# duyhominhnguyen/conan-fgw

Measured on AMD Instinct MI355X. Metric: molecules/s (K=5 conformers), higher is better.
Workload: dtype f32

## Files before the change

conan-fgw_amd/_lib.py:

```python
from __future__ import annotations

import ctypes
import os
import subprocess

import torch

_HERE = os.path.dirname(os.path.abspath(__file__))
_SO = os.path.join(_HERE, "libconan_fgw_hip.so")
_LIB = None
ABI_VERSION = 6

c_int, c_float, c_void_p, c_ll = ctypes.c_int, ctypes.c_float, ctypes.c_void_p, ctypes.c_longlong
f32, i32, i64 = torch.float32, torch.int32, torch.int64


def _c(t: torch.Tensor) -> torch.Tensor:
    return t if t.is_contiguous() else t.contiguous()


class FgwParams(ctypes.Structure):
    _fields_ = [("alpha", c_float), ("epsilon", c_float), ("max_iter", c_int), ("tol", c_float), ("inner_tol", c_float),
                ("num_iter_max", c_int), ("stop_thr", c_float), ("fixed_structure", c_int), ("fixed_features", c_int),
                ("warmstart", c_int), ("loss_fun", c_int), ("cs_small_int", c_int)]
# ... 149 lines not shown
    "conan_sinkhorn_bwd_lds_resident": (c_int, [c_int, c_int]),
    "conan_sinkhorn_bwd": (c_int, [_P] * 7 + [c_int, c_int, c_int, c_ll, c_float, c_int, c_int] + [_P] * 9),
    "conan_sinkhorn_ext_workspace_bytes": (c_ll, [c_int, c_int, c_int]),
    "conan_sinkhorn_ext_lds_resident": (c_int, [c_int, c_int]),
    "conan_sinkhorn_ext_nerr": (c_int, [c_int, c_int, c_int]),
    "conan_sinkhorn_ext_fwd": (c_int, [_P] * 7 + [c_int, c_int, c_int, c_ll, ctypes.c_double, c_int, c_int, ctypes.c_double, ctypes.c_double, c_int,
                                       ctypes.c_double, c_int] + [_P] * 11),
    "conan_fgw_barycenter_bwd": (c_int, [_P, _P, _P, _P, c_int, c_int, c_int, c_int, _P, _P]),
    "conan_fgw_barycenter_bwd_full_workspace_bytes": (c_ll, [c_int, c_int, c_int, c_int]),
    "conan_fgw_barycenter_bwd_full": (c_int, [_P, _P, _P, _P, _P, _P, _P, _P, _P, c_int, c_int, c_int, c_int, c_int, c_int, c_int,
                                              _P, _P, _P, _P, _P, _P, _P, _P]),
    "conan_fgw_readout_fwd": (c_int, [_P, c_int, c_int, c_int, c_int, c_int, _P, _P]),
    "conan_fgw_readout_bwd": (c_int, [_P, _P, c_int, c_int, c_int, c_int, c_int, _P, _P]),
}

_D = ctypes.c_double
EXT_SIGNATURES = {
    "conan_fgw_acc_pair_bwd_lds_resident": (c_int, [c_int]),
    "conan_fgw_acc_pair_bwd_workspace_bytes": (c_ll, [c_int, c_int, c_int]),
    "conan_fgw_acc_pair_bwd": (c_int, [_P] * 6 + [c_int, c_int, _D, _D, c_int] + [_P] * 12),
}

EXT_TABLES = {
    "conan_fgw_hip_pair_grad.h": {
        "conan_fgw_pair_bwd_lds_resident": (c_int, [c_int]),
        "conan_fgw_pair_bwd_workspace_bytes": (c_ll, [c_int, c_int, c_int, c_int]),
        "conan_fgw_pair_bwd": (c_int, [_P] * 6 + [c_int, c_int, _D, _D, c_int, c_int, _D, c_int, c_int] + [_P] * 13),
    },
    "conan_fgw_hip_bregman_grad.h": {
        "conan_fgw_bregman_bwd_lds_resident": (c_int, [c_int]),
        "conan_fgw_bregman_bwd_workspace_bytes": (c_ll, [c_int, c_int, c_int]),
        "conan_fgw_bregman_bwd": (c_int, [_P] * 6 + [c_int, c_int, _D, _D, c_int, c_int, c_int] + [_P] * 13),
    },
    "conan_fgw_hip_sinkhorn_hists.h": {
        "conan_sinkhorn_hists_max_hists": (c_int, [c_int, c_int]),
        "conan_sinkhorn_hists_lds_resident": (c_int, [c_int, c_int, c_int]),
        "conan_sinkhorn_hists_workspace_bytes": (c_ll, [c_int, c_int, c_int, c_int]),
        "conan_sinkhorn_hists_fwd": (c_int, [_P] * 8 + [c_int] * 4 + [c_ll, _D, c_int, _D] + [_P] * 7),
        "conan_sinkhorn_hists_loss_bwd": (c_int, [_P] * 7 + [c_int] * 4 + [c_ll, _D] + [_P] * 2),
    },
    "conan_fgw_hip_mixup_grad.h": {
        "conan_fgw_mixup_barycenter_fwd_record": (c_int, [_P] * 7 + [c_int, c_int, c_int, c_int, ctypes.POINTER(FgwParams), _D, c_int, _D] + [_P] * 9),
        "conan_fgw_mixup_barycenter_bwd_lds_resident": (c_int, [c_int]),
        "conan_fgw_mixup_barycenter_bwd_workspace_bytes": (c_ll, [c_int] * 5),
        "conan_fgw_mixup_barycenter_bwd": (c_int, [_P] * 6 + [c_int, c_int, c_int, c_int, ctypes.POINTER(FgwParams), _D, c_int, _D] + [_P] * 15),
    },
}

_ERR = {-1: "bad argument", -2: "HIP launch failure", -3: "unsupported configuration"}


def library_path() -> str:
    return _SO


def build(force: bool = False) -> str:
    args = ["make", "-C", os.path.join(_HERE, "csrc"), "-s", "-j8"]
    if force:
        args.append("-B")
    subprocess.check_call(args)
    return _SO


def lib():
    global _LIB
    if _LIB is None:
# ... 58 lines not shown
```

conan-fgw_amd/csrc/gemm.hip:

```cpp
#include "fp_planes.h"

namespace {

constexpr int BM = 64;
constexpr int BK = 32;
constexpr int XP = BK + 1;

template <int NB>
__global__ void __launch_bounds__(256) k_linear(const float *__restrict__ x, const float *__restrict__ w,
                                                const float *__restrict__ bias, const float *__restrict__ residual,
                                                int M, int K, int N, int w_kn, int act, float *__restrict__ y,
                                                const int *__restrict__ m_dev) {
    constexpr int BN = 64 * NB;
    if (m_dev) M = min(M, *m_dev);
    if ((int)blockIdx.x * BM >= M) return;
    constexpr int WP = BN + 1;
    __shared__ float xs[BM * XP];
    __shared__ float ws[BK * WP];
    const int tid = threadIdx.x, lane = tid & 63, wave = tid >> 6;
    const int wm = wave >> 1, wn = wave & 1;
    const int row0 = blockIdx.x * BM, col0 = blockIdx.y * BN;
    f32x16 acc[NB];
#pragma unroll
    for (int b = 0; b < NB; ++b)
#pragma unroll
        for (int r = 0; r < 16; ++r) acc[b][r] = 0.f;

    for (int k0 = 0; k0 < K; k0 += BK) {
        for (int t = tid; t < BM * BK; t += 256) {
            int r = t / BK, k = t % BK;
            int gr = row0 + r, gk = k0 + k;
            xs[r * XP + k] = (gr < M && gk < K) ? x[(size_t)gr * K + gk] : 0.f;
        }
// ... 167 lines not shown
                    if (act == 1) v = ssp_f(v);
                    if (act == 3) v = v / (1.0f + __expf(-v));
                    if (act == 2) v *= 1.0f - 0.5f * __expf(-rv[a][b][r]);
                    else if (residual) v += rv[a][b][r];
                    y[(size_t)gr * N + gc] = v;
                }
        }
    }
}

__global__ void k_ssp_bwd(const float *__restrict__ dy, const float *__restrict__ y, long long n, int width,
                          const int *__restrict__ m_dev, float *__restrict__ g) {
    if (m_dev) n = min(n, (long long)(*m_dev) * width);
    long long i = (long long)blockIdx.x * blockDim.x + threadIdx.x;
    const long long stride = (long long)gridDim.x * blockDim.x;
    for (; i < n; i += stride) g[i] = dy[i] * (1.0f - 0.5f * expf(-y[i]));
}

constexpr int WG_SLICES_MAX = 768;


__device__ __forceinline__ f32x16 wg_mma6(const bf16x8 &a1, const bf16x8 &a2, const bf16x8 &a3, const bf16x8 &b1, const bf16x8 &b2,
                                         const bf16x8 &b3, f32x16 acc) {
    acc = __builtin_amdgcn_mfma_f32_32x32x16_bf16(a3, b1, acc, 0, 0, 0);
    acc = __builtin_amdgcn_mfma_f32_32x32x16_bf16(a2, b2, acc, 0, 0, 0);
    acc = __builtin_amdgcn_mfma_f32_32x32x16_bf16(a1, b3, acc, 0, 0, 0);
    acc = __builtin_amdgcn_mfma_f32_32x32x16_bf16(a2, b1, acc, 0, 0, 0);
    acc = __builtin_amdgcn_mfma_f32_32x32x16_bf16(a1, b2, acc, 0, 0, 0);
    acc = __builtin_amdgcn_mfma_f32_32x32x16_bf16(a1, b1, acc, 0, 0, 0);
    return acc;
}


template <int KT, bool RBF, bool H16 = false>
__device__ __forceinline__ void wgrad_lds_body(const float *__restrict__ g, const float *__restrict__ x, int M, int K, int N,
                                               float *__restrict__ slabs, float *__restrict__ bias_slabs,
                                               const int *__restrict__ m_dev, const float *__restrict__ dist,
                                               const float *__restrict__ offset, float coeff, int slice, int num_slices, int tile_n, int tile_k,
                                               const float *__restrict__ gmax = nullptr) {
    constexpr int ROWS = 16, RG = ROWS / 8, W = 128 + KT, FRAGS = RG * W, NF = (FRAGS + 255) / 256;
    constexpr int TNB = KT == 128 ? 2 : 1;
    constexpr int NPL = H16 ? 2 : 3;
    static_assert(W % 64 == 0, "a wave's 64 fragments share one row group and one operand");
    __shared__ uint4 frag[2][NPL][RG][W];
    if (m_dev) M = min(M, *m_dev);
    float gsc = 1.0f, gun = 1.0f;
    if constexpr (H16) grad_scale(*gmax, 0.f, gsc, gun);
    const int tid = threadIdx.x, lane = tid & 63, wave = __builtin_amdgcn_readfirstlane(tid >> 6);
    const int l31 = lane & 31, h = lane >> 5;
    const int n0 = KT == 128 ? (wave >> 1) * 64 : wave * 32, k0 = KT == 128 ? (wave & 1) * 64 : 0;
    const int nb = tile_n * 128, kb = tile_k * KT;
    const int r_begin = slice * ROWS, r_end = M, STEP = num_slices * ROWS;
    f32x16 acc[TNB][2];
#pragma unroll
    for (int a = 0; a < TNB; ++a)
#pragma unroll
        for (int b = 0; b < 2; ++b)
#pragma unroll
            for (int r = 0; r < 16; ++r) acc[a][b][r] = 0.f;

    int f_rg[NF], f_col[NF];
    unsigned f_ldc[NF];
    bool f_act[NF], f_isg[NF], f_all[NF], f_on[NF];
    float f_off[NF], bsum[NF];
#pragma unroll
    for (int i = 0; i < NF; ++i) {
        const int fb = 64 * wave + 256 * i;
        f_act[i] = fb < FRAGS;
        f_rg[i] = fb / W;
        const int cb = fb - f_rg[i] * W;
        f_col[i] = cb + lane;
        f_isg[i] = cb < 128;
        const int cc = f_isg[i] ? nb + f_col[i] : kb + f_col[i] - 128;
        f_on[i] = cc < (f_isg[i] ? N : K);
        f_all[i] = __builtin_amdgcn_ballot_w64(f_on[i]) == ~0ull;
        f_ldc[i] = f_on[i] ? (unsigned)cc : 0u;
        f_off[i] = (RBF && !f_isg[i] && f_on[i]) ? offset[cc] : 0.f;
        bsum[i] = 0.f;
    }
    float stA[NF][8], stB[NF][8];
    auto fetch = [&](float (&st)[NF][8], int m0) {
        const bool full = m0 + ROWS <= r_end;
#pragma unroll
        for (int i = 0; i < NF; ++i) {
            if (!f_act[i]) continue;
            const int mr = m0 + 8 * f_rg[i];
            if (RBF && !f_isg[i]) {
#pragma unroll
                for (int j = 0; j < 8; ++j) st[i][j] = dist[full ? mr + j : min(mr + j, r_end - 1)];
            } else {
                const float *src = f_isg[i] ? g : x;
                const int ld = f_isg[i] ? N : K;
#pragma unroll
                for (int j = 0; j < 8; ++j) {
                    const int m = full ? mr + j : min(mr + j, r_end - 1);
                    st[i][j] = (src + (size_t)m * ld)[f_ldc[i]];
                }
            }
        }
    };
    auto stash = [&](int buf, float (&st)[NF][8], int m0) {
        const bool full = m0 + ROWS <= r_end;
#pragma unroll
        for (int i = 0; i < NF; ++i) {
            if (!f_act[i]) continue;
            if (RBF && !f_isg[i]) {
#pragma unroll
                for (int j = 0; j < 8; ++j) { const float t = st[i][j] - f_off[i]; st[i][j] = exp_neg_f(coeff * (t * t)); }
            }
            if (!full || !f_all[i]) {
#pragma unroll
                for (int j = 0; j < 8; ++j) st[i][j] = (f_on[i] && (m0 + 8 * f_rg[i] + j < r_end)) ? st[i][j] : 0.f;
            }
            if (f_isg[i]) bsum[i] += ((st[i][0] + st[i][1]) + (st[i][2] + st[i][3])) + ((st[i][4] + st[i][5]) + (st[i][6] + st[i][7]));
            if constexpr (H16) {
                const float sc = f_isg[i] ? gsc : 1.0f;
                f16x8 p1, p2;
                split2h(st[i], sc, p1, p2);
                frag[buf][0][f_rg[i]][f_col[i]] = __builtin_bit_cast(uint4, p1);
                frag[buf][1][f_rg[i]][f_col[i]] = __builtin_bit_cast(uint4, p2);
                continue;
            }
// ... 101 lines not shown
    wgrad_lds_body<KT, RBF>(g, x, M, K, N, slabs, bias_slabs, m_dev, dist, offset, coeff, blockIdx.x, gridDim.x, blockIdx.y, blockIdx.z);
}
__global__ void __launch_bounds__(256, 2) k_wgrad_lds_h16(const float *__restrict__ g, const float *__restrict__ x, int M, int K, int N,
                                                          float *__restrict__ slabs, float *__restrict__ bias_slabs, const int *__restrict__ m_dev,
                                                          const float *__restrict__ gmax) {
    wgrad_lds_body<128, false, true>(g, x, M, K, N, slabs, bias_slabs, m_dev, nullptr, nullptr, 0.f, blockIdx.x, gridDim.x, blockIdx.y, blockIdx.z, gmax);
}

constexpr int WGS_BATCH = 24;
struct WgradSlabJobs {
    const float *g[WGS_BATCH], *x[WGS_BATCH];
    const int *m_dev[WGS_BATCH];
    float *slabs[WGS_BATCH], *bias_slabs[WGS_BATCH];
    int M[WGS_BATCH], K[WGS_BATCH], N[WGS_BATCH], slices[WGS_BATCH], tiles_n[WGS_BATCH], first[WGS_BATCH + 1];
    int gsz[WGS_BATCH];
    int count;
};
template <int KT>
__global__ void __launch_bounds__(256, KT == 128 ? 2 : 3) k_wgrad_lds_batch(const WgradSlabJobs J) {
    const int b = blockIdx.x;
    int j = 0;
    while (j + 1 < J.count && b >= J.first[j + 1]) ++j;
    const int local = b - J.first[j];
    if (J.gsz[j] > 1) {
        const int gs = J.gsz[j], lo = local & 7, q = local >> 3, jm = j - (gs - 1) + q % gs;
        wgrad_lds_body<KT, false>(J.g[jm], J.x[jm], J.M[jm], J.K[jm], J.N[jm], J.slabs[jm], J.bias_slabs[jm], J.m_dev[jm], nullptr, nullptr, 0.f,
                                  lo + 8 * (q / gs), J.slices[jm], 0, 0);
        return;
    }
    const int slice = local % J.slices[j], rest = local / J.slices[j];
    const int tile_n = rest % J.tiles_n[j], tile_k = rest / J.tiles_n[j];
    wgrad_lds_body<KT, false>(J.g[j], J.x[j], J.M[j], J.K[j], J.N[j], J.slabs[j], J.bias_slabs[j], J.m_dev[j], nullptr, nullptr, 0.f, slice,
                              J.slices[j], tile_n, tile_k);
}

template <int NJ>
struct WgShared {
    const float *g[NJ];
    float *slab[NJ], *bslab[NJ];
    const float *x;
    const int *m_dev;
    int M, ldg, slices;
    long long slab_pitch;
    int bias_pitch;
};
template <int NJ, int D, int NW>
__global__ void __launch_bounds__(64 * NW, (NJ == 2 && NW == 4) ? 2 : 1) k_wgrad_lds_shared(const WgShared<NJ> P) {
    constexpr int K = 128, ROWS = 16, RG = 2, W = 128 * (NJ + 1), FRAGS = RG * W, NT = 64 * NW, NF = FRAGS / NT, TNB = NW == 8 ? 1 : 2;
    static_assert(FRAGS % NT == 0, "whole fragments per thread");
    extern __shared__ __attribute__((aligned(16))) uint4 frag_sh[];
    auto frag = [&](int buf, int pl, int rg, int col) -> uint4 & { return frag_sh[((buf * 3 + pl) * RG + rg) * W + col]; };
    int M = P.M;
    if (P.m_dev) M = min(M, *P.m_dev);
    const int tid = threadIdx.x, lane = tid & 63, wave = __builtin_amdgcn_readfirstlane(tid >> 6);
    const int l31 = lane & 31, h = lane >> 5;
    const int n0 = (wave >> 1) * (32 * TNB), k0 = (wave & 1) * 64;
    const int slice = blockIdx.x, num_slices = P.slices;
    const int r_begin = slice * ROWS, r_end = M, STEP = num_slices * ROWS;
    f32x16 acc[NJ][TNB][2];
#pragma unroll
    for (int j = 0; j < NJ; ++j)
#pragma unroll
        for (int a = 0; a < TNB; ++a)
#pragma unroll
            for (int b = 0; b < 2; ++b)
#pragma unroll
// ... 412 lines not shown

int conan_rbf_wgrad(const float *g, const float *dist, int M, const float *offset, int num_gaussians, float coeff, int N,
                    const int *m_dev, float *dW, float *dbias, float *ws, void *stream) {
    if (!g || !dist || !offset || !dW || !ws || M < 0 || num_gaussians <= 0 || N <= 0) return CONAN_E_BADARG;
    return wgrad_launch(g, nullptr, M, num_gaussians, N, m_dev, dW, dbias, ws, as_stream(stream), dist, offset, coeff);
}

}

int conan_wgrad_reduce_now(const float *slabs, const float *bias_slabs, int slices, int NK, int N, float *dW, float *dbias, hipStream_t s) {
    if ((NK & 3) || (N & 3)) return CONAN_E_UNSUPPORTED;
    const int cols4 = NK / 4 + (dbias ? N / 4 : 0);
    k_wgrad_reduce4<<<(cols4 + 31) / 32, 256, 0, s>>>(reinterpret_cast<const float4 *>(slabs), reinterpret_cast<const float4 *>(bias_slabs), slices,
                                                     NK / 4, N / 4, reinterpret_cast<float4 *>(dW), reinterpret_cast<float4 *>(dbias));
    CONAN_LAUNCH_CHECK();
    return CONAN_OK;
}

extern "C" {

int conan_wgrad_batchable(int K, int N) { return (((long long)N * K) & 3) == 0 && (N & 3) == 0 ? 1 : 0; }

int conan_linear_wgrad_slabs(const float *g, const float *x, int M, int K, int N, const int *m_dev, float *ws, void *stream) {
    if (!g || !x || !ws || M < 0 || K <= 0 || N <= 0 || !conan_wgrad_batchable(K, N)) return CONAN_E_BADARG;
    return wgrad_launch(g, x, M, K, N, m_dev, nullptr, nullptr, ws, as_stream(stream), nullptr, nullptr, 0.f);
}

int conan_rbf_wgrad_slabs(const float *g, const float *dist, int M, const float *offset, int num_gaussians, float coeff, int N,
                          const int *m_dev, float *ws, void *stream) {
    if (!g || !dist || !offset || !ws || M < 0 || num_gaussians <= 0 || N <= 0 || !conan_wgrad_batchable(num_gaussians, N)) return CONAN_E_BADARG;
    return wgrad_launch(g, nullptr, M, num_gaussians, N, m_dev, nullptr, nullptr, ws, as_stream(stream), dist, offset, coeff);
}

int conan_linear_wgrad_slabs_batch(const conan_wgrad_slab_job *jobs, int num_jobs, void *stream) {
    if (num_jobs < 0 || (num_jobs && !jobs)) return CONAN_E_BADARG;
    hipStream_t s = as_stream(stream);
    for (int j = 0; j < num_jobs; ++j) {
        const conan_wgrad_slab_job &b = jobs[j];
        if (!b.g || !b.x || !b.ws || b.M < 0 || b.K <= 0 || b.N <= 0 || b.slices < 0 || !conan_wgrad_batchable(b.K, b.N)) return CONAN_E_BADARG;
    }
    for (int wide = 0; wide < 2; ++wide) {
        WgradSlabJobs J;
        J.count = 0; J.first[0] = 0;
        auto flush = [&]() {
            if (!J.count) return;
            if (wide) k_wgrad_lds_batch<128><<<J.first[J.count], 256, 0, s>>>(J);
            else k_wgrad_lds_batch<64><<<J.first[J.count], 256, 0, s>>>(J);
            J.count = 0; J.first[0] = 0;
        };
        for (int j = 0; j < num_jobs; ++j) {
            const conan_wgrad_slab_job &b = jobs[j];
            if ((b.K > 64) != (wide != 0)) continue;
            const int KT = wide ? 128 : 64;
            const int dflt = wgrad_slices(b.M, b.K), slices = (b.slices > 0 && b.slices <= dflt) ? b.slices : dflt;
            const int tn = (b.N + 127) / 128, tk = (b.K + KT - 1) / KT;
            int run = 1;
            if (tn == 1 && tk == 1 && (slices & 7) == 0 && b.M > 0)
                while (j + run < num_jobs && run < 4 && jobs[j + run].x == b.x && jobs[j + run].M == b.M && jobs[j + run].K == b.K && jobs[j + run].N == b.N &&
                       jobs[j + run].m_dev == b.m_dev && jobs[j + run].slices == b.slices)
                    ++run;
            if ((run == 2 || run == 3) && wide && b.K == 128 && b.N == 128 && b.M >= CONAN_WGRAD_SHARED_MIN_ROWS) {
                auto fill = [&](auto &P) {
                    for (int r = 0; r < run; ++r) { P.g[r] = jobs[j + r].g; P.slab[r] = jobs[j + r].ws; P.bslab[r] = jobs[j + r].ws + (size_t)slices * b.N * b.K; }
                    P.x = b.x; P.m_dev = b.m_dev; P.M = b.M; P.ldg = b.N; P.slices = slices; P.slab_pitch = (long long)b.N * b.K; P.bias_pitch = b.N;
                };
                if (run == 2) { WgShared<2> P; fill(P); launch_wgrad_shared<2>(P, s); }
                else { WgShared<3> P; fill(P); launch_wgrad_shared<3>(P, s); }
                j += run - 1;
                continue;
            }
            if (J.count + run > WGS_BATCH) flush();
            for (int r = 0; r < run; ++r) {
                const conan_wgrad_slab_job &c = jobs[j + r];
                const int q = J.count;
                J.g[q] = c.g; J.x[q] = c.x; J.m_dev[q] = c.m_dev;
                J.slabs[q] = c.ws; J.bias_slabs[q] = c.ws + (size_t)slices * c.N * c.K;
                J.M[q] = c.M; J.K[q] = c.K; J.N[q] = c.N; J.slices[q] = slices; J.tiles_n[q] = tn;
                J.gsz[q] = (run > 1 && r == run - 1) ? run : 1;
                J.first[q + 1] = J.first[q] + ((run > 1 && r < run - 1) ? 0 : run * slices * tn * tk);
                ++J.count;
            }
            j += run - 1;
            if (J.count == WGS_BATCH) flush();
        }
        flush();
    }
    CONAN_LAUNCH_CHECK();
    return CONAN_OK;
}

int conan_wgrad_reduce_batch(const conan_wgrad_job *jobs, int num_jobs, void *stream) {
    if (num_jobs < 0 || (num_jobs && !jobs)) return CONAN_E_BADARG;
    hipStream_t s = as_stream(stream);
    for (int j0 = 0; j0 < num_jobs; j0 += WG_BATCH) {
        WgradJobs J;
        const int nb = num_jobs - j0 < WG_BATCH ? num_jobs - j0 : WG_BATCH;
        int max_cols4 = 0;
        for (int q = 0; q < nb; ++q) {
            const conan_wgrad_job &b = jobs[j0 + q];
            if (!b.ws || !b.dW || b.M < 0 || b.K <= 0 || b.N <= 0 || !conan_wgrad_batchable(b.K, b.N)) return CONAN_E_BADARG;
            const int slices = b.slices > 0 ? b.slices : wgrad_slices(b.M, b.K);
            const int NK = b.N * b.K;
            J.slabs[q] = reinterpret_cast<const float4 *>(b.ws);
            J.bias_slabs[q] = reinterpret_cast<const float4 *>(b.ws + (size_t)slices * NK);
            J.out[q] = reinterpret_cast<float4 *>(b.dW);
            J.bout[q] = reinterpret_cast<float4 *>(b.dbias);
            J.slices[q] = slices; J.NK4[q] = NK / 4; J.N4[q] = b.N / 4;
            const int cols4 = NK / 4 + (b.dbias ? b.N / 4 : 0);
            if (cols4 > max_cols4) max_cols4 = cols4;
        }
        for (int q = nb; q < WG_BATCH; ++q) { J.slabs[q] = J.bias_slabs[q] = nullptr; J.out[q] = J.bout[q] = nullptr; J.slices[q] = J.NK4[q] = J.N4[q] = 0; }
        k_wgrad_reduce4_batch<<<dim3((max_cols4 + 31) / 32, nb), 256, 0, s>>>(J);
    }
    CONAN_LAUNCH_CHECK();
    return CONAN_OK;
}

}
```

conan-fgw_amd/ops.py:

```python
from __future__ import annotations

from typing import Optional

import torch
from torch import Tensor

from . import wgrad
from ._lib import _c, call, f32, i32, i64, lib, ptr, stream_ptr


FUSED_GRAPH_BUILD = True


class RadiusGraph:

    def __init__(self, pos: Tensor, graph_ptr: Tensor, num_graphs: int, cutoff: float, max_num_neighbors: int, loop: bool = False,
                 pairs: bool = False, transpose: bool = False):
        pos = _c(pos)
        if pos.dtype != f32:
            raise RuntimeError("pos must be float32")
        n = pos.shape[0]
        dev = pos.device
        self.num_atoms, self.num_graphs, self.graph_ptr = n, num_graphs, graph_ptr
        self.cutoff, self.cap, self.loop = float(cutoff), int(max_num_neighbors), bool(loop)
# ... 420 lines not shown
        dx = torch.empty_like(y)
        call("conan_unary_bwd", ptr(y), ptr(_c(dy)), y.numel(), ctx.op, ptr(dx), stream_ptr())
        return dx, None


def relu(x: Tensor) -> Tensor:
    return _UnaryFn.apply(x, 0)


def sigmoid(x: Tensor) -> Tensor:
    return _UnaryFn.apply(x, 1)


def shifted_softplus(x: Tensor) -> Tensor:
    return _UnaryFn.apply(x, 2)


class _EmbeddingFn(torch.autograd.Function):
    @staticmethod
    def forward(ctx, z, weight, padding_idx):
        z, weight = _c(z), _c(weight)
        out = torch.empty(z.shape[0], weight.shape[1], dtype=f32, device=weight.device)
        call("conan_embedding_fwd", ptr(z, i64), ptr(weight, f32), z.shape[0], weight.shape[1], weight.shape[0], ptr(out), stream_ptr())
        ctx.save_for_backward(z, weight)
        ctx.shape, ctx.padding_idx = weight.shape, padding_idx
        return out

    @staticmethod
    def backward(ctx, dout):
        z, weight = ctx.saved_tensors
        rows, H = ctx.shape
        if rows <= 128 and wgrad.claim((weight.data_ptr(),), (H, rows), flush_if_pending=False):
            dout = _c(dout)
            onehot = torch.empty(z.shape[0], rows, dtype=f32, device=dout.device)
            call("conan_onehot_rows", ptr(z), z.shape[0], rows, -1 if ctx.padding_idx is None else ctx.padding_idx, ptr(onehot), stream_ptr())
            dw, _ = wgrad.plain(onehot, dout, z.shape[0], H, rows, None, weight, False)
            return None, dw, None
        dw = torch.empty(ctx.shape, dtype=f32, device=dout.device)
        ws = torch.empty(int(lib().conan_embedding_bwd_ws(z.shape[0], ctx.shape[1], ctx.shape[0])), dtype=f32, device=dout.device)
        call("conan_embedding_bwd", ptr(z), ptr(_c(dout)), z.shape[0], ctx.shape[1], ctx.shape[0],
             -1 if ctx.padding_idx is None else ctx.padding_idx, ptr(dw), ptr(ws), stream_ptr())
        return None, dw, None


def embedding(z: Tensor, weight: Tensor, padding_idx: Optional[int] = 0) -> Tensor:
    return _EmbeddingFn.apply(z, weight, padding_idx)


def rbf_expand(graph: RadiusGraph, offset: Tensor, coeff: float) -> Tensor:
    Gs = offset.shape[0]
    out = torch.empty(graph.max_edges, Gs, dtype=f32, device=offset.device)
    call("conan_rbf_fwd", ptr(graph.dist), ptr(graph.num_edges_dev), graph.max_edges, ptr(_c(offset), f32), Gs, float(coeff),
         ptr(out), stream_ptr())
    return out


class _CutoffScaleFn(torch.autograd.Function):
    @staticmethod
    def forward(ctx, w_raw, graph):
        out = torch.empty_like(w_raw)
        call("conan_cutoff_scale", ptr(graph.dist), ptr(graph.num_edges_dev), graph.max_edges, w_raw.shape[1], graph.cutoff,
             ptr(_c(w_raw)), ptr(out), stream_ptr())
        ctx.graph = graph
        return out

    @staticmethod
# ... 284 lines not shown
```

conan-fgw_amd/wgrad.py:

```python
import ctypes

import torch

from ._lib import WgradJob, WgradSlabJob, call, lib, ptr, stream_ptr

f32 = torch.float32
_LATE_STAGE1_ROWS = 65536
LATE_SLICES = 0
LATE_SLICES_AUTO = True


def _late_slices(n_jobs: int, M: int) -> int:
    dflt = max(1, (M + 127) // 128)
    if LATE_SLICES:
        return LATE_SLICES if LATE_SLICES < dflt else 0
    if not LATE_SLICES_AUTO:
        return 0
    s = 8 * max(1, round(1400 / max(1, min(n_jobs, 24)) / 8))
    return s if s < dflt else 0


class Job:
    __slots__ = ("ws", "dw_ptr", "db_ptr", "keep", "M", "K", "N", "slices", "weight_ptr", "stream", "operands")

    def __init__(self, ws, dw_ptr, db_ptr, keep, M, K, N, slices=0, weight_ptr=None, stream=None, operands=None):
        self.ws, self.dw_ptr, self.db_ptr, self.keep, self.M, self.K, self.N, self.slices = ws, dw_ptr, db_ptr, keep, M, K, N, slices
        self.weight_ptr, self.stream, self.operands = weight_ptr, stream, operands


_open = None
_flushed = {}


def pending():
    return None if _open is None else len(_open)


def flushed() -> dict:
    return _flushed


class deferred:
    def __enter__(self):
        global _open
        self._outermost, _open = _open is None, [] if _open is None else _open
        return self

    def __exit__(self, *exc):
        global _open
        if self._outermost:
            try:
                flush()
            finally:
                _open = None


def claim(weight_ptrs, shape=None, flush_if_pending=True) -> bool:
    if _open is None or (shape is not None and not lib().conan_wgrad_batchable(*shape)):
        return False
    twice = any(j.weight_ptr in weight_ptrs for j in _open)
    if twice and flush_if_pending:
        flush()
    return not twice


def job(ws, dw, db, M, K, N, weight_ptr, slices=0, operands=None) -> Job:
    return Job(ws, dw.data_ptr(), db.data_ptr() if db is not None else None, (dw.untyped_storage(), db.untyped_storage() if db is not None else None),
               M, K, N, slices, weight_ptr, torch.cuda.current_stream(), operands)


def slab_table(jobs, operands) -> ctypes.Array:
    return (WgradSlabJob * len(jobs))(*[WgradSlabJob(*map(ptr, o), ptr(j.ws), j.M, j.K, j.N, j.slices) for j, o in zip(jobs, operands)])


def reduce_table(jobs) -> ctypes.Array:
    return (WgradJob * len(jobs))(*[WgradJob(ptr(j.ws), j.dw_ptr, j.db_ptr, j.M, j.K, j.N, j.slices) for j in jobs])


def flush():
    if not _open:
        return {}
    cur = torch.cuda.current_stream()
    for st in {j.stream for j in _open} - {cur}:
        cur.wait_stream(st)
    late = [j for j in _open if j.operands is not None]
    if late:
        operands = [j.operands for j in late]
        for j in late:
            j.slices, j.operands = _late_slices(len(late), j.M), None
        call("conan_linear_wgrad_slabs_batch", slab_table(late, operands), len(late), stream_ptr())
        for t in {t for o in operands for t in o if t is not None}:
            t.record_stream(cur)
    call("conan_wgrad_reduce_batch", reduce_table(_open), len(_open), stream_ptr())
    done = {j.weight_ptr: (j.dw_ptr, j.db_ptr) for j in _open}
    for j in _open:
        j.ws.record_stream(cur)
    _open.clear()
    _flushed.update(done)
    return done


def plain(g, x, M, K, N, md, weight, has_bias, rbf=None, gmax=None):
    ws = torch.empty(int(lib().conan_linear_wgrad_ws(M, K, N)), dtype=f32, device=g.device)
    dw, db = torch.empty(N, K, dtype=f32, device=g.device), torch.empty(N, dtype=f32, device=g.device) if has_bias else None
    defer = claim((weight.data_ptr(),), (K, N))
    late = defer and rbf is None and M <= _LATE_STAGE1_ROWS and not (gmax is not None and K > 64)
    if rbf is not None:
        dist, offset, coeff = rbf
        if defer:
            call("conan_rbf_wgrad_slabs", ptr(g), ptr(dist), M, ptr(offset, f32), K, coeff, N, ptr(md), ptr(ws), stream_ptr())
        else:
            call("conan_rbf_wgrad", ptr(g), ptr(dist), M, ptr(offset, f32), K, coeff, N, ptr(md), ptr(dw), ptr(db), ptr(ws), stream_ptr())
    elif gmax is not None and K > 64:
        call("conan_linear_wgrad_scaled", ptr(g), ptr(x), M, K, N, ptr(md), None if defer else ptr(dw), None if defer else ptr(db), ptr(ws),
             ptr(gmax), stream_ptr())
    elif not defer:
        call("conan_linear_wgrad", ptr(g), ptr(x), M, K, N, ptr(md), ptr(dw), ptr(db), ptr(ws), stream_ptr())
    elif not late:
        call("conan_linear_wgrad_slabs", ptr(g), ptr(x), M, K, N, ptr(md), ptr(ws), stream_ptr())
    if defer:
        _open.append(job(ws, dw, db, M, K, N, weight.data_ptr(), operands=(g, x, md) if late else None))
    return dw, db


def shared_x(gs, x, M, K, N, md, weights, has_bias):
    n = len(gs)
    usable = n > 1 and bool(lib().conan_wgrad_batchable(K, N)) and K > 64 and N <= 128 and M > _LATE_STAGE1_ROWS
    wptrs = [w.data_ptr() for w in weights]
    if usable and _open is not None:
        usable = len(set(wptrs)) == n and claim(wptrs, flush_if_pending=False)
    if not usable:
        return [plain(g, x, M, K, N, md, w, hb) for g, w, hb in zip(gs, weights, has_bias)]
    dev, wsz = x.device, int(lib().conan_linear_wgrad_ws(M, K, N))
    wss = [torch.empty(wsz, dtype=f32, device=dev) for _ in range(n)]
    dws = [torch.empty(N, K, dtype=f32, device=dev) for _ in range(n)]
    dbs = [torch.empty(N, dtype=f32, device=dev) if hb else None for hb in has_bias]
    jobs = [job(wss[q], dws[q], dbs[q], M, K, N, wptrs[q]) for q in range(n)]
    call("conan_linear_wgrad_slabs_batch", slab_table(jobs, [(g, x, md) for g in gs]), n, stream_ptr())
    if _open is not None:
        _open.extend(jobs)
    else:
        call("conan_wgrad_reduce_batch", reduce_table(jobs), n, stream_ptr())
    return list(zip(dws, dbs))


def filter_bwd(g, h1, dist, offset, coeff, w1, w2, M, md, gmax=None):
    (F, Gs), dev = w1.shape, g.device
    ws = torch.empty(int(lib().conan_filter_bwd_ws(M, Gs, F)), dtype=f32, device=dev)
    dw, db = torch.empty(F, Gs, dtype=f32, device=dev), torch.empty(F, dtype=f32, device=dev)
    defer = claim((w1.data_ptr(),))
    call("conan_filter_bwd", ptr(g), ptr(h1), ptr(dist), M, ptr(offset, f32), Gs, coeff, ptr(w2), F, ptr(md),
         None if defer else ptr(dw), None if defer else ptr(db), ptr(ws), ptr(gmax), stream_ptr())
    if defer:
        _open.append(job(ws, dw, db, M, Gs, F, w1.data_ptr(), slices=int(lib().conan_filter_bwd_slices(M))))
    return dw, db


def filter_bwd2(g, h1, dist, offset, coeff, w1, w2, M, md, gmax):
    (F, Gs), dev = w1.shape, g.device
    ws = torch.empty(int(lib().conan_filter_bwd2_ws(M, Gs, F)), dtype=f32, device=dev)
    slices = int(lib().conan_filter_bwd2_slices(M))
    dw1, db1 = torch.empty(F, Gs, dtype=f32, device=dev), torch.empty(F, dtype=f32, device=dev)
    dw2, db2 = torch.empty(F, F, dtype=f32, device=dev), torch.empty(F, dtype=f32, device=dev)
    p1, p2 = w1.data_ptr(), w2.data_ptr()
    defer = claim((p1, p2))
    call("conan_filter_bwd2", ptr(g), ptr(h1), ptr(dist), M, ptr(offset, f32), Gs, coeff, ptr(w2), F, ptr(md), ptr(gmax),
         None if defer else ptr(dw1), None if defer else ptr(db1), None if defer else ptr(dw2), None if defer else ptr(db2), ptr(ws), stream_ptr())
    if defer:
        cut = slices * (F * Gs + F)
        _open.extend([job(ws[:cut], dw1, db1, M, Gs, F, p1, slices=slices), job(ws[cut:], dw2, db2, M, F, F, p2, slices=slices)])
    return (dw1, db1), (dw2, db2)
# ... 1 lines not shown
```

Baseline: 117,300.

## Batch weight-gradient slab jobs through a persistent worklist kernel

Replaces the two-launch (narrow/wide) batched wgrad slab path with one persistent grid-stride worklist kernel. The grid is sized to resident occupancy, work units are sorted by row stages, and each block walks a flattened list of slice/tile units across jobs, sharing an external LDS buffer. It also adds an optional path that generates embedding one-hot rows inside the kernel instead of materialising them, but that path is off by default. The goal is fewer launches and better load balance, at the cost of one kernel padded to KT=128 even for narrow jobs and extra per-item index lookup.

Result: no change. 116,600 (-0.6%).

```diff
diff --git a/conan-fgw_amd/_lib.py b/conan-fgw_amd/_lib.py
--- a/conan-fgw_amd/_lib.py
+++ b/conan-fgw_amd/_lib.py
@@ -205,6 +205,10 @@
         "conan_fgw_bregman_bwd_workspace_bytes": (c_ll, [c_int, c_int, c_int]),
         "conan_fgw_bregman_bwd": (c_int, [_P] * 6 + [c_int, c_int, _D, _D, c_int, c_int, c_int] + [_P] * 13),
     },
+    "conan_fgw_hip_wgrad_batch.h": {
+        "conan_linear_wgrad_slabs_worklist": (c_int, [ctypes.POINTER(WgradSlabJob), c_int, _P, _P, c_int, c_int, _P]),
+        "conan_wgrad_worklist_resident": (c_int, [c_int]),
+    },
     "conan_fgw_hip_sinkhorn_hists.h": {
         "conan_sinkhorn_hists_max_hists": (c_int, [c_int, c_int]),
         "conan_sinkhorn_hists_lds_resident": (c_int, [c_int, c_int, c_int]),
diff --git a/conan-fgw_amd/csrc/gemm.hip b/conan-fgw_amd/csrc/gemm.hip
--- a/conan-fgw_amd/csrc/gemm.hip
+++ b/conan-fgw_amd/csrc/gemm.hip
@@ -1,4 +1,7 @@
+#include <algorithm>
+#include <vector>
 #include "fp_planes.h"
+#include "../../include/conan_fgw_hip_wgrad_batch.h"
 
 namespace {
 
@@ -232,17 +235,25 @@
 }
 
 
-template <int KT, bool RBF, bool H16 = false>
+template <int KT, bool RBF, bool H16 = false, bool EXT = false, bool ONEHOT = false>
 __device__ __forceinline__ void wgrad_lds_body(const float *__restrict__ g, const float *__restrict__ x, int M, int K, int N,
                                                float *__restrict__ slabs, float *__restrict__ bias_slabs,
                                                const int *__restrict__ m_dev, const float *__restrict__ dist,
                                                const float *__restrict__ offset, float coeff, int slice, int num_slices, int tile_n, int tile_k,
-                                               const float *__restrict__ gmax = nullptr) {
+                                               const float *__restrict__ gmax = nullptr, uint4 *ext_lds = nullptr,
+                                               const long long *__restrict__ z = nullptr, int z_pad = -1) {
     constexpr int ROWS = 16, RG = ROWS / 8, W = 128 + KT, FRAGS = RG * W, NF = (FRAGS + 255) / 256;
     constexpr int TNB = KT == 128 ? 2 : 1;
     constexpr int NPL = H16 ? 2 : 3;
     static_assert(W % 64 == 0, "a wave's 64 fragments share one row group and one operand");
-    __shared__ uint4 frag[2][NPL][RG][W];
+    static_assert(!(ONEHOT && (RBF || H16)), "one generated operand at a time");
+    uint4 (*frag)[NPL][RG][W];
+    if constexpr (EXT) {
+        frag = reinterpret_cast<uint4 (*)[NPL][RG][W]>(ext_lds);
+    } else {
+        __shared__ uint4 own[2][NPL][RG][W];
+        frag = own;
+    }
     if (m_dev) M = min(M, *m_dev);
     float gsc = 1.0f, gun = 1.0f;
     if constexpr (H16) grad_scale(*gmax, 0.f, gsc, gun);
@@ -263,6 +274,7 @@
     unsigned f_ldc[NF];
     bool f_act[NF], f_isg[NF], f_all[NF], f_on[NF];
     float f_off[NF], bsum[NF];
+    [[maybe_unused]] bool f_hot[NF];
 #pragma unroll
     for (int i = 0; i < NF; ++i) {
         const int fb = 64 * wave + 256 * i;
@@ -277,6 +289,7 @@
         f_ldc[i] = f_on[i] ? (unsigned)cc : 0u;
         f_off[i] = (RBF && !f_isg[i] && f_on[i]) ? offset[cc] : 0.f;
         bsum[i] = 0.f;
+        if constexpr (ONEHOT) f_hot[i] = f_isg[i] && f_on[i] && cc != z_pad;
     }
     float stA[NF][8], stB[NF][8];
     auto fetch = [&](float (&st)[NF][8], int m0) {
@@ -288,6 +301,10 @@
             if (RBF && !f_isg[i]) {
 #pragma unroll
                 for (int j = 0; j < 8; ++j) st[i][j] = dist[full ? mr + j : min(mr + j, r_end - 1)];
+            } else if (ONEHOT && f_isg[i]) {
+#pragma unroll
+                for (int j = 0; j < 8; ++j)
+                    st[i][j] = (f_hot[i] && z[full ? mr + j : min(mr + j, r_end - 1)] == (long long)f_ldc[i]) ? 1.0f : 0.0f;
             } else {
                 const float *src = f_isg[i] ? g : x;
                 const int ld = f_isg[i] ? N : K;
@@ -455,6 +472,44 @@
     const int tile_n = rest % J.tiles_n[j], tile_k = rest / J.tiles_n[j];
     wgrad_lds_body<KT, false>(J.g[j], J.x[j], J.M[j], J.K[j], J.N[j], J.slabs[j], J.bias_slabs[j], J.m_dev[j], nullptr, nullptr, 0.f, slice,
                               J.slices[j], tile_n, tile_k);
+}
+
+struct WgradWorkJobs {
+    const float *g[WGS_BATCH], *x[WGS_BATCH];
+    const int *m_dev[WGS_BATCH];
+    const long long *z[WGS_BATCH];
+    float *slabs[WGS_BATCH], *bias_slabs[WGS_BATCH];
+    int M[WGS_BATCH], K[WGS_BATCH], N[WGS_BATCH], slices[WGS_BATCH], tiles_n[WGS_BATCH], first[WGS_BATCH + 1], gsz[WGS_BATCH], zpad[WGS_BATCH];
+    int count;
+};
+template <bool TWO_BODIES>
+__global__ void __launch_bounds__(256, 2) k_wgrad_worklist(const WgradWorkJobs J) {
+    __shared__ uint4 lds[2 * 3 * 2 * 256];
+    const int total = J.first[J.count];
+    for (int it = blockIdx.x; it < total; it += gridDim.x) {
+        if (it != (int)blockIdx.x) __syncthreads();
+        int j = 0;
+        while (j + 1 < J.count && it >= J.first[j + 1]) ++j;
+        const int local = it - J.first[j];
+        int jm = j, slice, tile_n = 0, tile_k = 0;
+        if (J.gsz[j] > 1) {
+            const int gs = J.gsz[j], lo = local & 7, q = local >> 3;
+            jm = j - (gs - 1) + q % gs;
+            slice = lo + 8 * (q / gs);
+        } else {
+            const int rest = local / J.slices[j];
+            slice = local % J.slices[j]; tile_n = rest % J.tiles_n[j]; tile_k = rest / J.tiles_n[j];
+        }
+        if (J.z[jm])
+            wgrad_lds_body<128, false, false, true, true>(nullptr, J.x[jm], J.M[jm], J.K[jm], J.N[jm], J.slabs[jm], J.bias_slabs[jm], J.m_dev[jm], nullptr,
+                                                          nullptr, 0.f, slice, J.slices[jm], tile_n, tile_k, nullptr, lds, J.z[jm], J.zpad[jm]);
+        else if (TWO_BODIES && J.K[jm] <= 64)
+            wgrad_lds_body<64, false, false, true>(J.g[jm], J.x[jm], J.M[jm], J.K[jm], J.N[jm], J.slabs[jm], J.bias_slabs[jm], J.m_dev[jm], nullptr, nullptr,
+                                                   0.f, slice, J.slices[jm], tile_n, tile_k, nullptr, lds);
+        else
+            wgrad_lds_body<128, false, false, true>(J.g[jm], J.x[jm], J.M[jm], J.K[jm], J.N[jm], J.slabs[jm], J.bias_slabs[jm], J.m_dev[jm], nullptr, nullptr,
+                                                    0.f, slice, J.slices[jm], tile_n, tile_k, nullptr, lds);
+    }
 }
 
 template <int NJ>
@@ -933,13 +988,33 @@
     return wgrad_launch(g, nullptr, M, num_gaussians, N, m_dev, nullptr, nullptr, ws, as_stream(stream), dist, offset, coeff);
 }
 
-int conan_linear_wgrad_slabs_batch(const conan_wgrad_slab_job *jobs, int num_jobs, void *stream) {
-    if (num_jobs < 0 || (num_jobs && !jobs)) return CONAN_E_BADARG;
-    hipStream_t s = as_stream(stream);
-    for (int j = 0; j < num_jobs; ++j) {
-        const conan_wgrad_slab_job &b = jobs[j];
-        if (!b.g || !b.x || !b.ws || b.M < 0 || b.K <= 0 || b.N <= 0 || b.slices < 0 || !conan_wgrad_batchable(b.K, b.N)) return CONAN_E_BADARG;
-    }
+}
+
+namespace {
+
+int wgrad_batch_run(const conan_wgrad_slab_job *jobs, int num_jobs, const long long *const *z, int j, int slices, int tn, int tk) {
+    const conan_wgrad_slab_job &b = jobs[j];
+    int run = 1;
+    if (tn == 1 && tk == 1 && (slices & 7) == 0 && b.M > 0 && !(z && z[j]))
+        while (j + run < num_jobs && run < 4 && jobs[j + run].x == b.x && jobs[j + run].M == b.M && jobs[j + run].K == b.K && jobs[j + run].N == b.N &&
+               jobs[j + run].m_dev == b.m_dev && jobs[j + run].slices == b.slices && !(z && z[j + run]))
+            ++run;
+    return run;
+}
+bool wgrad_batch_run_is_shared(const conan_wgrad_slab_job &b, int run) {
+    return (run == 2 || run == 3) && b.K == 128 && b.N == 128 && b.M >= CONAN_WGRAD_SHARED_MIN_ROWS;
+}
+void wgrad_batch_launch_shared(const conan_wgrad_slab_job *run_jobs, int run, int slices, hipStream_t s) {
+    const conan_wgrad_slab_job &b = run_jobs[0];
+    auto fill = [&](auto &P) {
+        for (int r = 0; r < run; ++r) { P.g[r] = run_jobs[r].g; P.slab[r] = run_jobs[r].ws; P.bslab[r] = run_jobs[r].ws + (size_t)slices * b.N * b.K; }
+        P.x = b.x; P.m_dev = b.m_dev; P.M = b.M; P.ldg = b.N; P.slices = slices; P.slab_pitch = (long long)b.N * b.K; P.bias_pitch = b.N;
+    };
+    if (run == 2) { WgShared<2> P; fill(P); launch_wgrad_shared<2>(P, s); }
+    else { WgShared<3> P; fill(P); launch_wgrad_shared<3>(P, s); }
+}
+
+void wgrad_batch_two_launches(const conan_wgrad_slab_job *jobs, int num_jobs, hipStream_t s) {
     for (int wide = 0; wide < 2; ++wide) {
         WgradSlabJobs J;
         J.count = 0; J.first[0] = 0;
@@ -955,18 +1030,9 @@
             const int KT = wide ? 128 : 64;
             const int dflt = wgrad_slices(b.M, b.K), slices = (b.slices > 0 && b.slices <= dflt) ? b.slices : dflt;
             const int tn = (b.N + 127) / 128, tk = (b.K + KT - 1) / KT;
-            int run = 1;
-            if (tn == 1 && tk == 1 && (slices & 7) == 0 && b.M > 0)
-                while (j + run < num_jobs && run < 4 && jobs[j + run].x == b.x && jobs[j + run].M == b.M && jobs[j + run].K == b.K && jobs[j + run].N == b.N &&
-                       jobs[j + run].m_dev == b.m_dev && jobs[j + run].slices == b.slices)
-                    ++run;
-            if ((run == 2 || run == 3) && wide && b.K == 128 && b.N == 128 && b.M >= CONAN_WGRAD_SHARED_MIN_ROWS) {
-                auto fill = [&](auto &P) {
-                    for (int r = 0; r < run; ++r) { P.g[r] = jobs[j + r].g; P.slab[r] = jobs[j + r].ws; P.bslab[r] = jobs[j + r].ws + (size_t)slices * b.N * b.K; }
-                    P.x = b.x; P.m_dev = b.m_dev; P.M = b.M; P.ldg = b.N; P.slices = slices; P.slab_pitch = (long long)b.N * b.K; P.bias_pitch = b.N;
-                };
-                if (run == 2) { WgShared<2> P; fill(P); launch_wgrad_shared<2>(P, s); }
-                else { WgShared<3> P; fill(P); launch_wgrad_shared<3>(P, s); }
+            const int run = wgrad_batch_run(jobs, num_jobs, nullptr, j, slices, tn, tk);
+            if (wide && wgrad_batch_run_is_shared(b, run)) {
+                wgrad_batch_launch_shared(jobs + j, run, slices, s);
                 j += run - 1;
                 continue;
             }
@@ -986,8 +1052,104 @@
         }
         flush();
     }
+}
+
+int wgrad_worklist_resident(bool two_bodies, hipStream_t s) {
+    static int cached[2] = {0, 0};
+    int &c = cached[two_bodies ? 1 : 0];
+    if (c > 0) return c;
+    hipStreamCaptureStatus st = hipStreamCaptureStatusNone;
+    if (hipStreamIsCapturing(s, &st) != hipSuccess || st != hipStreamCaptureStatusNone) return 0;
+    int dev = 0, cus = 0, per_cu = 0;
+    if (hipGetDevice(&dev) != hipSuccess || hipDeviceGetAttribute(&cus, hipDeviceAttributeMultiprocessorCount, dev) != hipSuccess) return 0;
+    const hipError_t e = two_bodies ? hipOccupancyMaxActiveBlocksPerMultiprocessor(&per_cu, k_wgrad_worklist<true>, 256, 0)
+                                    : hipOccupancyMaxActiveBlocksPerMultiprocessor(&per_cu, k_wgrad_worklist<false>, 256, 0);
+    if (e != hipSuccess || cus <= 0 || per_cu <= 0) return 0;
+    return c = cus * per_cu;
+}
+
+int wgrad_batch_worklist(const conan_wgrad_slab_job *jobs, int num_jobs, const long long *const *z, const int *zpad, bool two_bodies, int grid_cap,
+                         hipStream_t s) {
+    int resident = wgrad_worklist_resident(two_bodies, s);
+    if (resident <= 0) return CONAN_E_UNSUPPORTED;
+    if (grid_cap > 0 && grid_cap < resident) resident = grid_cap;
+    if (resident > 8) resident &= ~7;
+    struct Unit { int j, run, slices, tn, tk, stages; };
+    std::vector<Unit> units;
+    units.reserve(num_jobs);
+    for (int j = 0; j < num_jobs; ++j) {
+        const conan_wgrad_slab_job &b = jobs[j];
+        const int dflt = wgrad_slices(b.M, b.K), slices = (b.slices > 0 && b.slices <= dflt) ? b.slices : dflt;
+        const int tn = (b.N + 127) / 128, tk = (b.K + 127) / 128;
+        const int run = wgrad_batch_run(jobs, num_jobs, z, j, slices, tn, tk);
+        if (b.K > 64 && wgrad_batch_run_is_shared(b, run)) wgrad_batch_launch_shared(jobs + j, run, slices, s);
+        else units.push_back({j, run, slices, tn, tk, (b.M + 16 * slices - 1) / (16 * slices)});
+        j += run - 1;
+    }
+    std::stable_sort(units.begin(), units.end(), [](const Unit &a, const Unit &b) { return a.stages > b.stages; });
+    WgradWorkJobs J;
+    J.count = 0; J.first[0] = 0;
+    auto flush = [&]() {
+        if (!J.count) return;
+        const int total = J.first[J.count], grid = total < resident ? total : resident;
+        if (two_bodies) k_wgrad_worklist<true><<<grid, 256, 0, s>>>(J);
+        else k_wgrad_worklist<false><<<grid, 256, 0, s>>>(J);
+        J.count = 0; J.first[0] = 0;
+    };
+    for (const Unit &u : units) {
+        if (J.count + u.run > WGS_BATCH) flush();
+        for (int r = 0; r < u.run; ++r) {
+            const conan_wgrad_slab_job &c = jobs[u.j + r];
+            const int q = J.count;
+            J.g[q] = c.g; J.x[q] = c.x; J.m_dev[q] = c.m_dev;
+            J.z[q] = z ? z[u.j + r] : nullptr; J.zpad[q] = (z && zpad) ? zpad[u.j + r] : -1;
+            J.slabs[q] = c.ws; J.bias_slabs[q] = c.ws + (size_t)u.slices * c.N * c.K;
+            J.M[q] = c.M; J.K[q] = c.K; J.N[q] = c.N; J.slices[q] = u.slices; J.tiles_n[q] = u.tn;
+            J.gsz[q] = (u.run > 1 && r == u.run - 1) ? u.run : 1;
+            J.first[q + 1] = J.first[q] + ((u.run > 1 && r < u.run - 1) ? 0 : u.run * u.slices * u.tn * u.tk);
+            ++J.count;
+        }
+        if (J.count == WGS_BATCH) flush();
+    }
+    flush();
+    return CONAN_OK;
+}
+
+}
+
+extern "C" {
+
+int conan_wgrad_worklist_resident(int form) {
+    if (form != CONAN_WGRAD_BATCH_WORKLIST && form != CONAN_WGRAD_BATCH_WORKLIST_TWO_BODIES) return CONAN_E_BADARG;
+    return wgrad_worklist_resident(form == CONAN_WGRAD_BATCH_WORKLIST_TWO_BODIES, nullptr);
+}
+
+int conan_linear_wgrad_slabs_worklist(const conan_wgrad_slab_job *jobs, int num_jobs, const long long *const *z, const int *padding_idx, int form,
+                                      int grid_cap, void *stream) {
+    if (num_jobs < 0 || (num_jobs && !jobs) || form < CONAN_WGRAD_BATCH_TWO_LAUNCHES || form > CONAN_WGRAD_BATCH_WORKLIST_TWO_BODIES || grid_cap < 0)
+        return CONAN_E_BADARG;
+    hipStream_t s = as_stream(stream);
+    bool any_z = false;
+    for (int j = 0; j < num_jobs; ++j) {
+        const conan_wgrad_slab_job &b = jobs[j];
+        const bool hot = z && z[j];
+        if ((!b.g && !hot) || !b.x || !b.ws || b.M < 0 || b.K <= 0 || b.N <= 0 || b.slices < 0 || !conan_wgrad_batchable(b.K, b.N)) return CONAN_E_BADARG;
+        any_z = any_z || hot;
+    }
+    if (!num_jobs) return CONAN_OK;
+    int rc = CONAN_E_UNSUPPORTED;
+    if (form != CONAN_WGRAD_BATCH_TWO_LAUNCHES)
+        rc = wgrad_batch_worklist(jobs, num_jobs, z, padding_idx, form == CONAN_WGRAD_BATCH_WORKLIST_TWO_BODIES, grid_cap, s);
+    if (rc == CONAN_E_UNSUPPORTED) {
+        if (any_z) return CONAN_E_UNSUPPORTED;
+        wgrad_batch_two_launches(jobs, num_jobs, s);
+    }
     CONAN_LAUNCH_CHECK();
     return CONAN_OK;
+}
+
+int conan_linear_wgrad_slabs_batch(const conan_wgrad_slab_job *jobs, int num_jobs, void *stream) {
+    return conan_linear_wgrad_slabs_worklist(jobs, num_jobs, nullptr, nullptr, CONAN_WGRAD_BATCH_WORKLIST, 0, stream);
 }
 
 int conan_wgrad_reduce_batch(const conan_wgrad_job *jobs, int num_jobs, void *stream) {
diff --git a/conan-fgw_amd/ops.py b/conan-fgw_amd/ops.py
--- a/conan-fgw_amd/ops.py
+++ b/conan-fgw_amd/ops.py
@@ -476,6 +476,8 @@
         rows, H = ctx.shape
         if rows <= 128 and wgrad.claim((weight.data_ptr(),), (H, rows), flush_if_pending=False):
             dout = _c(dout)
+            if wgrad.onehot_in_kernel(z.shape[0]):
+                return None, wgrad.onehot_late(z, ctx.padding_idx, dout, z.shape[0], H, rows, weight), None
             onehot = torch.empty(z.shape[0], rows, dtype=f32, device=dout.device)
             call("conan_onehot_rows", ptr(z), z.shape[0], rows, -1 if ctx.padding_idx is None else ctx.padding_idx, ptr(onehot), stream_ptr())
             dw, _ = wgrad.plain(onehot, dout, z.shape[0], H, rows, None, weight, False)
diff --git a/conan-fgw_amd/wgrad.py b/conan-fgw_amd/wgrad.py
--- a/conan-fgw_amd/wgrad.py
+++ b/conan-fgw_amd/wgrad.py
@@ -8,6 +8,8 @@
 _LATE_STAGE1_ROWS = 65536
 LATE_SLICES = 0
 LATE_SLICES_AUTO = True
+BATCH_FORM = 1
+ONEHOT_IN_KERNEL = False
 
 
 def _late_slices(n_jobs: int, M: int) -> int:
@@ -21,11 +23,12 @@
 
 
 class Job:
-    __slots__ = ("ws", "dw_ptr", "db_ptr", "keep", "M", "K", "N", "slices", "weight_ptr", "stream", "operands")
+    __slots__ = ("ws", "dw_ptr", "db_ptr", "keep", "M", "K", "N", "slices", "weight_ptr", "stream", "operands", "onehot")
 
-    def __init__(self, ws, dw_ptr, db_ptr, keep, M, K, N, slices=0, weight_ptr=None, stream=None, operands=None):
+    def __init__(self, ws, dw_ptr, db_ptr, keep, M, K, N, slices=0, weight_ptr=None, stream=None, operands=None, onehot=None):
         self.ws, self.dw_ptr, self.db_ptr, self.keep, self.M, self.K, self.N, self.slices = ws, dw_ptr, db_ptr, keep, M, K, N, slices
         self.weight_ptr, self.stream, self.operands = weight_ptr, stream, operands
+        self.onehot = onehot
 
 
 _open = None
@@ -64,13 +67,21 @@
     return not twice
 
 
-def job(ws, dw, db, M, K, N, weight_ptr, slices=0, operands=None) -> Job:
+def job(ws, dw, db, M, K, N, weight_ptr, slices=0, operands=None, onehot=None) -> Job:
     return Job(ws, dw.data_ptr(), db.data_ptr() if db is not None else None, (dw.untyped_storage(), db.untyped_storage() if db is not None else None),
-               M, K, N, slices, weight_ptr, torch.cuda.current_stream(), operands)
+               M, K, N, slices, weight_ptr, torch.cuda.current_stream(), operands, onehot)
 
 
 def slab_table(jobs, operands) -> ctypes.Array:
     return (WgradSlabJob * len(jobs))(*[WgradSlabJob(*map(ptr, o), ptr(j.ws), j.M, j.K, j.N, j.slices) for j, o in zip(jobs, operands)])
+
+
+def slabs_batch(jobs, operands, onehots=None, grid_cap=0):
+    z = pad = None
+    if onehots is not None and any(o is not None for o in onehots):
+        z = (ctypes.c_void_p * len(jobs))(*[None if o is None else ptr(o[0], torch.int64) for o in onehots])
+        pad = (ctypes.c_int * len(jobs))(*[-1 if o is None else int(o[1]) for o in onehots])
+    call("conan_linear_wgrad_slabs_worklist", slab_table(jobs, operands), len(jobs), z, pad, int(BATCH_FORM), int(grid_cap), stream_ptr())
 
 
 def reduce_table(jobs) -> ctypes.Array:
@@ -85,11 +96,11 @@
         cur.wait_stream(st)
     late = [j for j in _open if j.operands is not None]
     if late:
-        operands = [j.operands for j in late]
+        operands, onehots = [j.operands for j in late], [j.onehot for j in late]
         for j in late:
-            j.slices, j.operands = _late_slices(len(late), j.M), None
-        call("conan_linear_wgrad_slabs_batch", slab_table(late, operands), len(late), stream_ptr())
-        for t in {t for o in operands for t in o if t is not None}:
+            j.slices, j.operands, j.onehot = _late_slices(len(late), j.M), None, None
+        slabs_batch(late, operands, onehots)
+        for t in {t for o in operands for t in o if t is not None} | {o[0] for o in onehots if o is not None}:
             t.record_stream(cur)
     call("conan_wgrad_reduce_batch", reduce_table(_open), len(_open), stream_ptr())
     done = {j.weight_ptr: (j.dw_ptr, j.db_ptr) for j in _open}
@@ -98,6 +109,17 @@
     _open.clear()
     _flushed.update(done)
     return done
+
+
+def onehot_in_kernel(M: int) -> bool:
+    return bool(ONEHOT_IN_KERNEL) and BATCH_FORM != 0 and M <= _LATE_STAGE1_ROWS
+
+
+def onehot_late(z, padding_idx, x, M, K, N, weight):
+    ws = torch.empty(int(lib().conan_linear_wgrad_ws(M, K, N)), dtype=f32, device=x.device)
+    dw = torch.empty(N, K, dtype=f32, device=x.device)
+    _open.append(job(ws, dw, None, M, K, N, weight.data_ptr(), operands=(None, x, None), onehot=(z, -1 if padding_idx is None else padding_idx)))
+    return dw
 
 
 def plain(g, x, M, K, N, md, weight, has_bias, rbf=None, gmax=None):
@@ -136,7 +158,7 @@
     dws = [torch.empty(N, K, dtype=f32, device=dev) for _ in range(n)]
     dbs = [torch.empty(N, dtype=f32, device=dev) if hb else None for hb in has_bias]
     jobs = [job(wss[q], dws[q], dbs[q], M, K, N, wptrs[q]) for q in range(n)]
-    call("conan_linear_wgrad_slabs_batch", slab_table(jobs, [(g, x, md) for g in gs]), n, stream_ptr())
+    slabs_batch(jobs, [(g, x, md) for g in gs])
     if _open is not None:
         _open.extend(jobs)
     else:
diff --git a/include/conan_fgw_hip_wgrad_batch.h b/include/conan_fgw_hip_wgrad_batch.h
--- /dev/null
+++ b/include/conan_fgw_hip_wgrad_batch.h
@@ -0,0 +1,21 @@
+#ifndef CONAN_FGW_HIP_WGRAD_BATCH_H
+#define CONAN_FGW_HIP_WGRAD_BATCH_H
+
+#include "conan_fgw_hip.h"
+
+#ifdef __cplusplus
+extern "C" {
+#endif
+
+#define CONAN_WGRAD_BATCH_TWO_LAUNCHES 0
+#define CONAN_WGRAD_BATCH_WORKLIST 1
+#define CONAN_WGRAD_BATCH_WORKLIST_TWO_BODIES 2
+
+int conan_linear_wgrad_slabs_worklist(const conan_wgrad_slab_job *jobs, int num_jobs, const long long *const *z, const int *padding_idx, int form,
+                                      int grid_cap, void *stream);
+int conan_wgrad_worklist_resident(int form);
+
+#ifdef __cplusplus
+}
+#endif
+#endif
```
